# SafeRL-Lab/Massive-MARL-Benchmark

Measured on AMD Instinct MI355X. Metric: env-steps/sec (whole node), TenAnt 4096 envs/GPU, PPO rollout, higher is better.
Workload: dtype f32 (policy-layer products: fp32 operands as 2 row-scaled fp16 planes (kept to 2^-22), 3 f16 MFMA products, fp32 accumulation; error vs float64 <= the exact-fp32 MFMA kernel's, see policy_layers_error_vs_f64); 1 GPU; TenAnt num_envs=4096 per GPU, PPO rollout: ActorCritic MLP [1024,1024,512]x2 (fp32) + fused sim step (dt 0.0166, 2 substeps) + RolloutStorage + GAE every 8 steps; envs_per_gpu=4096, global_envs=4096, parallelism=env-sharded x1, no data-path collective, hipgraph=True, refresh_in_graph=True, rollouts_per_graph=1, fused_act_and_bound_slots=True, obs_planes_from_step_kernel=True, policy_head_in_step_kernel=True, critic_stream=True, critic_deferred=False, finite=True, resets_total=97569

## Files before the change

massive_marl_benchmark_amd/algorithms/rl/ppo/module.py:

```python
import ctypes
import math

import numpy as np
import torch
import torch.nn as nn

from .... import _lib


def get_activation(act_name):
    table = {"elu": nn.ELU, "selu": nn.SELU, "relu": nn.ReLU, "crelu": nn.ReLU, "lrelu": nn.LeakyReLU, "tanh": nn.Tanh,
             "sigmoid": nn.Sigmoid}
    if act_name not in table:
        print("invalid activation function!")
        return None
    return table[act_name]()


def _mlp(in_dim, hidden, out_dim, activation):
    layers, d = [], in_dim
    for h in hidden:
        layers += [nn.Linear(d, h), activation]
        d = h
    layers.append(nn.Linear(d, out_dim))
# ... 318 lines not shown
                continue
            x_planes[g0] = (bufs["x"][g0], bufs["xi"][g0], bufs["cs"][g0], bufs["ci"][g0])
            calls.append((L.mms_split_planes16_group, (idx, 1, M, x.shape[1], x.stride(0), arr([x]), arr([bufs["x"][g0]]), arr([bufs["xs"][g0]]), arr([bufs["xi"][g0]]),
                                                       nch, Lh if nch else 0, arr([chain]) if nch else None, arr([bufs["cs"][g0]]) if nch else None,
                                                       arr([bufs["ci"][g0]]) if nch else None, None, 0.0), "mms_split_planes16_group"))
            bufs["keep"].append(x)
        cur = [x_planes[src[g][0]][0] for g in range(G)]
        cur_inv = [x_planes[src[g][0]][1] for g in range(G)]
        for li in range(nl):
            last = li == nl - 1
            out = bufs["out"] if last else bufs["h"][li]
            ysc = None if last else arr([x_planes[src[g][0]][2][src[g][1], li] for g in range(G)])
            calls.append((L.mms_linear_group_act_split16, (idx, G, M, recs[0][li]["N"], recs[0][li]["K"], arr(cur), arr([recs[g][li]["planes"] for g in range(G)]),
                                                           arr([recs[g][li]["lin"].bias for g in range(G)]), arr(out), arr(cur_inv),
                                                           arr([recs[g][li]["inv"] for g in range(G)]), ysc, 1, 0 if last else 1, None, None, None, None, None, 0),
                          "mms_linear_group_act_split16"))
            if not last:
                cur, cur_inv = out, [x_planes[src[g][0]][3][src[g][1], li] for g in range(G)]
        return calls, bufs["out"]

    def _split_applies(self, M, lins, networks=2):
        if not (self.split_layers and M > 0 and M % 128 == 0 and all(l.out_features % 128 == 0 for l in lins)):
            return False
        need = self.split_min_tiles
        if need is None:
            dev = lins[0].weight.device
            need = torch.cuda.get_device_properties(dev).multi_processor_count if dev.type == "cuda" else 1
        return max(networks * (M // 128) * (l.out_features // 128) for l in lins) >= need

    def _split_hidden(self, nets, inputs, tag, planes=None):
        if self.split_format == "f16x2":
            return self._split_hidden16(nets, inputs, tag, planes)
        assert self.split_format == "bf16x3", self.split_format
        self._ensure_fresh()
        x0 = inputs[0]
        dev, M, K = x0.device, x0.shape[0], x0.shape[1]
        L, idx, stream = _lib.for_device(dev)
        G, nl = len(nets), len(nets[0])
        key = (tag, M, K, str(dev), G, tuple(l.out_features for l in nets[0]))
        if self._split_bufs is None:
            self._split_bufs = {}
        bufs = self._split_bufs.get(key)
        if bufs is None:
            u8 = lambda n: torch.empty(n, dtype=torch.uint8, device=dev)
            bufs = {"x": [u8(self._p32_bytes(M, K)) for _ in range(G)],
                    "h": [[u8(self._p32_bytes(M, l.out_features)) for _ in range(G)] for l in nets[0][:-1]],
                    "out": [torch.empty(M, nets[0][-1].out_features, device=dev) for _ in range(G)]}
            self._split_bufs[key] = bufs
        arr = lambda ts: (ctypes.c_void_p * len(ts))(*[t.data_ptr() for t in ts])
        cur = []
        for g, x in enumerate(inputs):
            same = next((h for h in range(g) if inputs[h].data_ptr() == x.data_ptr() and inputs[h].shape == x.shape), None)
            if same is not None:
                cur.append(cur[same])
                continue
            assert x.dtype == torch.float32 and x.stride(1) == 1
            _lib.check(L.mms_split_planes(idx, M, K, x.stride(0), ctypes.c_void_p(x.data_ptr()), ctypes.c_void_p(bufs["x"][g].data_ptr()), stream),
                       None, "mms_split_planes", L)
            cur.append(bufs["x"][g])
        for li in range(nl):
            lins = [net[li] for net in nets]
            last = li == nl - 1
            out = bufs["out"] if last else bufs["h"][li]
            wp = [self._weight_planes(l, L, idx, stream) for l in lins]
            _lib.check(L.mms_linear_group_act_split(idx, G, M, lins[0].out_features, lins[0].in_features, arr(cur), arr(wp),
                                                    arr([l.bias.detach() for l in lins]), arr(out), 1, 0 if last else 1, None, None, None, None, None, 0, stream),
                       None, "mms_linear_group_act_split", L)
            cur = out
        return bufs["out"]

    def _fused_hidden(self, x, critic_in, planes=None):
        a_lin = [m for m in self.actor if isinstance(m, nn.Linear)]
        c_lin = [m for m in self.critic if isinstance(m, nn.Linear)]
        if not self._fp32_layers_qualify():
            return None
        p = lambda t: ctypes.c_void_p(t.data_ptr())
        dev = x.device
        L, idx, stream = _lib.for_device(dev)
        ha, hc = x.contiguous(), critic_in.contiguous()
        M = ha.shape[0]
        if self._split_applies(M, a_lin[:-1]) and ha.data_ptr() % 16 == 0 and hc.data_ptr() % 16 == 0:
            out = self._split_hidden([a_lin[:-1], c_lin[:-1]], [ha, hc], "act", planes)
            return out[0], out[1]
        key = (M, str(dev))
        if self._act_bufs is None or self._act_bufs[0] != key:
            self._act_bufs = (key, [(torch.empty(M, la.out_features, device=dev), torch.empty(M, la.out_features, device=dev))
                                    for la in a_lin[:-1]])
        for (la, lc), (ya, yc) in zip(zip(a_lin[:-1], c_lin[:-1]), self._act_bufs[1]):
            _lib.check(L.mms_linear2_act(idx, M, la.out_features, la.in_features, p(ha), p(la.weight.detach()), p(la.bias.detach()), p(ya),
                                         p(hc), p(lc.weight.detach()), p(lc.bias.detach()), p(yc), 1, stream), None, "mms_linear2_act", L)
            ha, hc = ya, yc
        return ha, hc

    def _hidden_one(self, net, x):
        lin = [m for m in net if isinstance(m, nn.Linear)][:-1]
        L, idx, stream = _lib.for_device(x.device)
        p = lambda t: ctypes.c_void_p(t.data_ptr())
        M = x.shape[0]
        key = (M, str(x.device), id(net))
        if self._one_bufs is None or self._one_bufs[0] != key:
            self._one_bufs = (key, [torch.empty(M, l.out_features, device=x.device) for l in lin])
        h = x
        for l, y in zip(lin, self._one_bufs[1]):
            _lib.check(L.mms_linear2_act(idx, M, l.out_features, l.in_features, p(h), p(l.weight.detach()), p(l.bias.detach()), p(y),
                                         None, None, None, None, 1, stream), None, "mms_linear2_act", L)
            h = y
        return h

    def _actor_pass(self, x):
        last = self.actor[-1]
        if (self.fuse_head and x.is_cuda and isinstance(last, nn.Linear) and last.weight.dtype == torch.float32
                and last.in_features % 64 == 0 and last.out_features <= 128 and last.bias is not None):
            if self._trunk is None:
                self._trunk = [self.actor[:-1]]
            return None, self._trunk[0](x)
        return self.actor(x), None

    def _sample(self, mean, value, hidden=None, vhidden=None):
        src = mean if mean is not None else hidden
        N, A = src.shape[0], self.log_std.shape[0]
        dev = src.device
        L, idx, stream = _lib.for_device(dev)
        if self._counters is None or self._counters.numel() != N or self._counters.device != dev:
            self._counters = torch.zeros(N, dtype=torch.int64, device=dev)
        storage, actions_out = self._bound if self._bound is not None else (None, None)
        ckey = None
        if storage is not None and mean is None and value is None and hidden.is_contiguous() and (vhidden is None or vhidden.is_contiguous()):
            la, lc = self.actor[-1], self.critic[-1]
            ckey = (storage.actions.data_ptr(), storage.values.data_ptr(), storage.step, hidden.data_ptr(), None if vhidden is None else vhidden.data_ptr(),
                    None if actions_out is None else actions_out.data_ptr(), N, la.weight.data_ptr(), la.bias.data_ptr(), lc.weight.data_ptr(),
                    lc.bias.data_ptr(), self.log_std.data_ptr(), self._counters.data_ptr(), None if self._step_engine is None else id(self._step_engine))
            if self._sample_calls is None:
                self._sample_calls = {}
            hit = self._sample_calls.get(ckey)
            if hit is not None:
                args, ret, head = hit
                if head is not None and self._step_engine is not None:
                    self._step_engine.bind_policy_head(head)
                else:
                    _lib.check(L.mms_ppo_heads_act(*args, stream), None, "mms_ppo_heads_act", L)
                return ret
        if storage is not None:
            s = storage.step
            act, logp, val = storage.actions[s], storage.actions_log_prob[s], storage.values[s]
            mu, sigma = storage.mu[s], storage.sigma[s]
        else:
            act, mu, sigma = (torch.empty(N, A, device=dev) for _ in range(3))
            logp, val = torch.empty(N, 1, device=dev), torch.empty(N, 1, device=dev)
        p = lambda t: None if t is None else ctypes.c_void_p(t.data_ptr())
        value = None if value is None else value.contiguous().float()
        log_std = self.log_std.detach().float().contiguous()
        if mean is not None:
            mean = mean.contiguous().float()
            _lib.check(L.mms_ppo_act(idx, p(mean), p(value), p(log_std), self.seed, p(self._counters), self.row_offset, 1,
                                     p(actions_out), p(act), p(logp), p(val), p(mu), p(sigma), N, A, stream),
                       None, "mms_ppo_act", L)
        else:
            last = self.actor[-1]
            hidden = hidden.contiguous()
            vlast = self.critic[-1]
            vh = None if vhidden is None else vhidden.contiguous()
            args = (idx, p(hidden), p(last.weight.detach()), p(last.bias.detach()), last.in_features, p(value), p(vh),
                    None if vh is None else p(vlast.weight.detach()), None if vh is None else p(vlast.bias.detach()),
                    0 if vh is None else vlast.in_features, p(log_std), self.seed, p(self._counters), self.row_offset, 1,
                    p(actions_out), p(act), p(logp), p(val), p(mu), p(sigma), N, A)
            head = None
# ... 106 lines not shown
```

massive_marl_benchmark_amd/csrc/head_block.h:

```cpp
#pragma once
#include <hip/hip_runtime.h>
#ifndef MMS_HEAD_STAMP
#define MMS_HEAD_STAMP 0
#endif
#include <stdint.h>

#include "mms_lane.h"
#include "rollout_lane.h"

namespace mms {

struct PpoActOut {
    float* actions_out; float* act_slot; float* logp_slot; float* value_slot; float* mu_slot; float* sigma_slot;
    float* lds_actions = nullptr;
    int64_t lds_row0 = 0;
};
__device__ __forceinline__ void ppo_sample_row(const float* mean_row, const float* __restrict__ value, const float* __restrict__ log_std,
                                               uint64_t seed, int64_t* __restrict__ counters, int64_t row_offset, int ref_scale,
                                               const PpoActOut& o, int64_t row, int A, int lane, bool have_value = false, float value_now = 0.f) {
    const int64_t c = counters[row];
    float lp = 0.f;
    for (int j = lane; j < A; j += 64) {
        const float ls = log_std[j];
        const float m = mean_row[j];
        float term;
        const float act = ppo_sample_one(m, ls, seed, (uint64_t)(row_offset + row), (uint64_t)c, (uint32_t)j, ref_scale, term);
        lp += term;
        if (o.actions_out) o.actions_out[row * A + j] = act;
        if (o.lds_actions) o.lds_actions[(row - o.lds_row0) * A + j] = act;
        if (o.act_slot) o.act_slot[row * A + j] = act;
        if (o.mu_slot) o.mu_slot[row * A + j] = m;
        if (o.sigma_slot) o.sigma_slot[row * A + j] = ls;
    }
#pragma unroll
    for (int m = 32; m >= 1; m >>= 1) lp += __shfl_xor(lp, m, 64);
    if (lane == 0) {
        if (o.logp_slot) o.logp_slot[row] = lp;
        if (o.value_slot && (have_value || value)) o.value_slot[row] = have_value ? value_now : value[row];
        counters[row] = c + 1;
    }
}

typedef float f32x4 __attribute__((ext_vector_type(4)));

template <int NCT, int WAVES, int RT, int UB = 4, bool TILED = false>
__device__ __forceinline__ void ppo_head_block(float* s_part, const int tid, const bool active, const int64_t r0,
                                               const float* __restrict__ hidden, const float* __restrict__ weight,
                                               const float* __restrict__ bias, int H, const float* __restrict__ value,
                                               const float* __restrict__ vhidden, const float* __restrict__ vweight,
                                               const float* __restrict__ vbias, int VH,
                                               const float* __restrict__ log_std, uint64_t seed, int64_t* __restrict__ counters,
                                               int64_t row_offset, int ref_scale, const PpoActOut& o, int64_t N, int A,
                                               const float* __restrict__ weight_tiles = nullptr) {
    constexpr int AP = NCT * 16, ROWS = 16 * RT;
    constexpr int RPW = ROWS / WAVES;
#if MMS_HEAD_STAMP
    uint64_t st[6];
    st[0] = __builtin_amdgcn_s_memrealtime();
#define MMS_HEAD_ST(i) do { asm volatile("s_waitcnt vmcnt(0) lgkmcnt(0)" ::: "memory"); st[i] = __builtin_amdgcn_s_memrealtime(); } while (0)
#else
#define MMS_HEAD_ST(i) do { } while (0)
#endif
    const int lane = tid & 63, wave = active ? (tid >> 6) : 0;
    const int i = lane & 15, g = lane >> 4;
    float v_rows[RPW];
#pragma unroll
    for (int q = 0; q < RPW; q++) v_rows[q] = 0.f;
    if (active) {
        const float* hrow[RT];
#pragma unroll
        for (int rt = 0; rt < RT; rt++) {
            const int64_t row_a = r0 + 16 * rt + i < N ? r0 + 16 * rt + i : N - 1;
            hrow[rt] = hidden + row_a * (int64_t)H + 4 * g;
        }
        const float* wrow[NCT];
#pragma unroll
        for (int ct = 0; ct < NCT; ct++) {
            const int j = ct * 16 + i;
            wrow[ct] = weight + (int64_t)(j < A ? j : A - 1) * H + 4 * g;
        }
        f32x4 acc[RT][NCT];
#pragma unroll
        for (int rt = 0; rt < RT; rt++)
#pragma unroll
            for (int ct = 0; ct < NCT; ct++) acc[rt][ct] = f32x4{0.f, 0.f, 0.f, 0.f};
#pragma unroll
        for (int q = 0; q < RPW; q++) {
            const int64_t row = r0 + wave * RPW + q;
            if (vhidden && row < N) {
                const float* hv = vhidden + row * (int64_t)VH;
                float part = 0.f;
                for (int k = lane * 4; k < VH; k += 256) {
                    const float4 h4 = *reinterpret_cast<const float4*>(hv + k), w4 = *reinterpret_cast<const float4*>(vweight + k);
                    part += h4.x * w4.x + h4.y * w4.y + h4.z * w4.z + h4.w * w4.w;
                }
#pragma unroll
                for (int m = 32; m >= 1; m >>= 1) part += __shfl_xor(part, m, 64);
                v_rows[q] = part + vbias[0];
            }
        }
        MMS_HEAD_ST(1);
        const int kq = H / WAVES;
        const int kbeg = wave * kq;
        for (int kc = kbeg; kc < kbeg + kq; kc += 64) {
#pragma unroll
            for (int u0 = 0; u0 < 4; u0 += UB) {
                float4 a[RT][UB], b[UB][NCT];
#pragma unroll
                for (int u = 0; u < UB; u++) {
#pragma unroll
                    for (int rt = 0; rt < RT; rt++) a[rt][u] = *reinterpret_cast<const float4*>(hrow[rt] + kc + 16 * (u0 + u));
#pragma unroll
                    for (int ct = 0; ct < NCT; ct++)
                        b[u][ct] = TILED ? *reinterpret_cast<const float4*>(weight_tiles + ((size_t)(ct * (H / 4) + (kc / 4 + 4 * (u0 + u) + g)) * 16 + i) * 4)
                                         : *reinterpret_cast<const float4*>(wrow[ct] + kc + 16 * (u0 + u));
                }
#pragma unroll
                for (int rt = 0; rt < RT; rt++)
#pragma unroll
                    for (int u = 0; u < UB; u++) {
#pragma unroll
                        for (int ct = 0; ct < NCT; ct++) acc[rt][ct] = __builtin_amdgcn_mfma_f32_16x16x4f32(a[rt][u].x, b[u][ct].x, acc[rt][ct], 0, 0, 0);
#pragma unroll
                        for (int ct = 0; ct < NCT; ct++) acc[rt][ct] = __builtin_amdgcn_mfma_f32_16x16x4f32(a[rt][u].y, b[u][ct].y, acc[rt][ct], 0, 0, 0);
#pragma unroll
                        for (int ct = 0; ct < NCT; ct++) acc[rt][ct] = __builtin_amdgcn_mfma_f32_16x16x4f32(a[rt][u].z, b[u][ct].z, acc[rt][ct], 0, 0, 0);
#pragma unroll
                        for (int ct = 0; ct < NCT; ct++) acc[rt][ct] = __builtin_amdgcn_mfma_f32_16x16x4f32(a[rt][u].w, b[u][ct].w, acc[rt][ct], 0, 0, 0);
                    }
            }
        }
        MMS_HEAD_ST(2);
        float* mine = s_part + (size_t)wave * ROWS * AP;
#pragma unroll
        for (int rt = 0; rt < RT; rt++)
#pragma unroll
            for (int ct = 0; ct < NCT; ct++) {
#pragma unroll
                for (int r = 0; r < 4; r++) mine[(16 * rt + 4 * g + r) * AP + ct * 16 + i] = acc[rt][ct][r];
            }
    }
    __syncthreads();
    MMS_HEAD_ST(3);
    float* s_mean = s_part + (size_t)WAVES * ROWS * AP;
    if (active)
        for (int e = tid; e < ROWS * AP; e += 64 * WAVES) {
            const int j = e % AP;
            float sum = s_part[e];
#pragma unroll
            for (int w = 1; w < WAVES; w++) sum += s_part[w * ROWS * AP + e];
            s_mean[e] = sum + bias[j < A ? j : 0];
        }
    __syncthreads();
    MMS_HEAD_ST(4);
    if (active) {
#pragma unroll
        for (int q = 0; q < RPW; q++) {
            const int r = wave * RPW + q;
            const int64_t row = r0 + r;
            if (row >= N) continue;
            ppo_sample_row(s_mean + r * AP, value, log_std, seed, counters, row_offset, ref_scale, o, row, A, lane, vhidden != nullptr, v_rows[q]);
        }
    }
#if MMS_HEAD_STAMP
    MMS_HEAD_ST(5);
    if (r0 == 0 && tid == 0 && o.sigma_slot)
        for (int i = 1; i < 6; i++) o.sigma_slot[i] = 0.01f * (float)(st[i] - st[0]);
#endif
}

}
```

massive_marl_benchmark_amd/csrc/rollout_lane.h:

```cpp
#pragma once
#include "mms_lane.h"

namespace mms {

MMS_HD void gae_ppo_column(const float* rewards, const uint8_t* dones, const float* values, const float* last_values, float* returns,
                           float* advantages, int T, int64_t N, int64_t i, float gamma, float lam, double& sum, double& sq) {
    float adv = 0.f;
    float next_v = last_values[i];
    for (int t = T - 1; t >= 0; t--) {
        float v = values[t * N + i];
        float nt = 1.0f - (float)dones[t * N + i];
        float delta = rewards[t * N + i] + nt * gamma * next_v - v;
        adv = delta + nt * gamma * lam * adv;
        float ret = adv + v;
        returns[t * N + i] = ret;
        float a = ret - v;
        advantages[t * N + i] = a;
        sum += (double)a;
        sq += (double)a * (double)a;
        next_v = v;
    }
}
MMS_HD void adv_norm_params(const double* stats, float& mean, float& inv) {
    double n = stats[2];
    double m = stats[0] / n;
    double var = (stats[1] - n * m * m) / (n - 1.0);
    inv = (float)(1.0 / (sqrt(var > 0.0 ? var : 0.0) + 1e-8));
    mean = (float)m;
}
MMS_HD void gae_marl_column(const float* rewards, const float* value_preds, const float* masks, float* returns, int T, int64_t N, int64_t cols,
                            int64_t c, int64_t i, float gamma, float lam, int use_norm, float mean, float var) {
    float sd = 1.f;
    if (use_norm) sd = sqrtf(var); else mean = 0.f;
    float gae = 0.f;
    float v1 = value_preds[(int64_t)T * cols + c];
    if (use_norm) v1 = v1 * sd + mean;
    for (int t = T - 1; t >= 0; t--) {
        float v0 = value_preds[(int64_t)t * cols + c];
        if (use_norm) v0 = v0 * sd + mean;
        float m = masks[(int64_t)(t + 1) * N + i];
        float delta = rewards[(int64_t)t * N + i] + gamma * v1 * m - v0;
        gae = delta + gamma * lam * m * gae;
        returns[(int64_t)t * cols + c] = gae + v0;
        v1 = v0;
    }
}
MMS_HD int64_t marl_view_source(int64_t i, int agents, int per, int shared) {
    const int w = per + shared, row = agents * per + shared;
    int64_t e = i / ((int64_t)agents * w);
    int r = (int)(i - e * agents * w);
    int k = r / w, j = r - k * w;
    int src = (j < per) ? k * per + j : agents * per + (j - per);
    return e * row + src;
}
MMS_HD float ppo_sample_one(float mean, float log_std, uint64_t seed, uint64_t row_global, uint64_t counter, uint32_t j, int ref_scale, float& logp_term) {
    float scale, lscale;
    if (ref_scale) { float sd = expf(log_std); scale = sd * sd; lscale = logf(scale); }
    else { scale = expf(log_std); lscale = log_std; }
    const float z = rand_normal(seed, row_global, counter, j);
    logp_term = -0.5f * z * z - lscale - 0.9189385332046727f;
    return mean + scale * z;
}

}
```

massive_marl_benchmark_amd/csrc/step_kernels.hip:

```cpp
#include <hip/hip_runtime.h>

#include "head_block.h"
#include "mms_lane.h"
#include "step_args.h"

namespace mms {

template <int CTRL>
__device__ __forceinline__ float dpp_mov(float x) {
    return __builtin_bit_cast(float, __builtin_amdgcn_update_dpp(0, __builtin_bit_cast(int, x), CTRL, 0xF, 0xF, true));
}
__device__ __forceinline__ float quad_sum(float x) {
    x += dpp_mov<0xB1>(x);
    x += dpp_mov<0x4E>(x);
    return x;
}
__device__ __forceinline__ float oct_sum(float x) {
    x = quad_sum(x);
    x += dpp_mov<0x141>(x);
    return x;
}
__device__ __forceinline__ void quad_sum(Sym6& A, S6& p) {
#pragma unroll
    for (int k = 0; k < 21; k++) A.m[k] = quad_sum(A.m[k]);
// ... 4 lines not shown
#pragma unroll
    for (int k = 0; k < 9; k++) c.t[k] = oct_sum(c.t[k]);
}
__device__ __forceinline__ float wave_sum(float x) {
    x = oct_sum(x);
    x += dpp_mov<0x140>(x);
    x += __shfl_xor(x, 16, 64);
    x += __shfl_xor(x, 32, 64);
    return x;
}

typedef float f32x4_t __attribute__((ext_vector_type(4)));
__device__ __forceinline__ void stream_store(float4* dst, float4 v) {
    __builtin_nontemporal_store(f32x4_t{v.x, v.y, v.z, v.w}, reinterpret_cast<f32x4_t*>(dst));
}

__device__ __forceinline__ RigidState load_rigid(const float* r) {
    RigidState B;
    B.pos = V3{r[0], r[1], r[2]};
    B.qx = r[3]; B.qy = r[4]; B.qz = r[5]; B.qw = r[6];
    B.vel = V3{r[7], r[8], r[9]};
    B.ang = V3{r[10], r[11], r[12]};
    return B;
}
__device__ __forceinline__ void store_rigid(float* r, const RigidState& B) {
    r[0] = B.pos.x; r[1] = B.pos.y; r[2] = B.pos.z;
    r[3] = B.qx; r[4] = B.qy; r[5] = B.qz; r[6] = B.qw;
    r[7] = B.vel.x; r[8] = B.vel.y; r[9] = B.vel.z;
    r[10] = B.ang.x; r[11] = B.ang.y; r[12] = B.ang.z;
}

#ifndef MMS_WAVES_PER_EU
#define MMS_WAVES_PER_EU 2
#endif
__host__ __device__ inline size_t ant_env_lds_floats(int obs_dim, int A) {
    return (size_t)((obs_dim + 3) & ~3) + 16 + (sizeof(BoxPose) + 15) / 16 * 4 + 28 + 8 + (size_t)(((RP_STRIDE + 6) * A + 3) & ~3) +
           (size_t)((4 * A + 2 + 7 + 3) & ~3);
}
#ifndef MMS_WAVES_PER_EU_PACKED
#define MMS_WAVES_PER_EU_PACKED 3
#endif
template <int TASK, int BLOCK, int EPB, int AT, bool DR, bool HEAD = false>
#ifndef MMS_WAVES_PER_EU_WIDE
#define MMS_WAVES_PER_EU_WIDE 3
#endif
__global__ void __launch_bounds__(BLOCK, BLOCK == 64 ? MMS_WAVES_PER_EU : ((BLOCK == 192 || BLOCK == 768) ? MMS_WAVES_PER_EU_PACKED : MMS_WAVES_PER_EU_WIDE)) ant_step_kernel(StepArgs a) {
    extern __shared__ __attribute__((aligned(16))) float lds[];
    const mms_config* __restrict__ Cg = a.cfg;
    constexpr int kCfgFloats = (int)((sizeof(mms_config) + 15) / 16 * 4);
    static_assert(sizeof(mms_config) % 4 == 0, "copied word by word");
    const mms_config* C = reinterpret_cast<const mms_config*>(lds);
    const mms_model* M = &C->model;
    float2 ac_head = make_float2(0.f, 0.f);
    constexpr int kObsAT = TASK == MMS_TASK_TEN_ANT ? 38 * AT + 8 : (TASK == MMS_TASK_MULTI_ANT_CIRCLE ? 38 * AT : 60);
    constexpr int kPrevAT = TASK == MMS_TASK_TEN_ANT ? 4 * AT + 2 : (TASK == MMS_TASK_MULTI_ANT_CIRCLE ? 2 * AT : 6);
    const int obs_dim = AT > 0 ? kObsAT : a.obs_dim;
    const int prev_dim = AT > 0 ? kPrevAT : a.prev_dim;
    const int obs_pad = (obs_dim + 3) & ~3;

    const int A = AT > 0 ? AT : a.num_agents;
    const int LA = 4 * A;
    const int ant_region = EPB * LA;
    const int box_region = (BLOCK == 512 && EPB == 1 && ant_region <= 448) ? 448 : ((ant_region + 7) & ~7);
    const int bt = (int)threadIdx.x - box_region;
    const bool is_ant = (int)threadIdx.x < ant_region;
    const bool is_box = bt >= 0 && bt < 8 * EPB;
    const int e_loc = EPB == 1 ? 0 : (is_ant ? (int)threadIdx.x / LA : (is_box ? bt >> 3 : 0));
    const int tid = is_ant ? (int)threadIdx.x - e_loc * LA : 0;
    const int corner = bt & 7;
    const bool box_lead = is_box && corner == 0;
    const int env_raw = blockIdx.x * EPB + e_loc;
    const bool live = env_raw < a.num_envs;
    const int env = live ? env_raw : a.num_envs - 1;
    const int ant = tid >> 2, leg = tid & 3;

    LegConst* s_leg = reinterpret_cast<LegConst*>(lds + kCfgFloats);
    constexpr int kBoxOff = 0, kBpOff = 16, kFacOff = kBpOff + (int)((sizeof(BoxPose) + 15) / 16 * 4), kEpiOff = kFacOff + 28, kRedOff = kEpiOff + 8;
    const size_t env_stride = (ant_env_lds_floats(obs_dim, A) + 3) & ~(size_t)3;
    float* lds_envs = lds + kCfgFloats + (4 * sizeof(LegConst) + 15) / 16 * 4;
    float* s_root = lds_envs + (size_t)EPB * ((ant_env_lds_floats(AT > 0 ? kObsAT : a.obs_dim, A) + 3) & ~(size_t)3);
    constexpr bool kStage = AT > 0 && ((EPB * (AT + 1) * 13) % 4) == 0;
    const int root_floats = kStage ? EPB * (A + 1) * 13 : 0;
    float* lds_lanes = s_root + ((root_floats + 3) & ~3);
    if constexpr (HEAD) {
        static_assert(BLOCK == 768 && EPB == 16 && AT == 10 && TASK == MMS_TASK_TEN_ANT && kStage, "the fused head assumes 16 rows x 80 actions per block");
        float* s_head = lds_lanes;
        float* s_head_actions = s_head + 9 * 16 * 80;
        static_assert((9 + 1) * 16 * 80 <= 6 * 4 * BLOCK, "the head's LDS must fit the parking space");
        if (threadIdx.x >= 512) {
            const int t = (int)threadIdx.x - 512;
            const float4* src = reinterpret_cast<const float4*>(a.root_states + (size_t)blockIdx.x * root_floats);
            for (int i = t; i < root_floats / 4; i += 256) reinterpret_cast<float4*>(s_root)[i] = src[i];
            for (int i = t; i < (int)(sizeof(mms_config) / 4); i += 256) lds[i] = reinterpret_cast<const float*>(Cg)[i];
            if (t < 4) s_leg[t] = load_leg_const(&Cg->model, t);
            constexpr int kStageOff = ((kRedOff + (RP_STRIDE + 6) * AT + 3) & ~3) + ((kObsAT + 3) & ~3);
            for (int i = t; i < EPB * prev_dim; i += 256) {
                const int e = i / prev_dim, k = i - e * prev_dim;
                (lds_envs + (size_t)e * env_stride + kStageOff)[k] = a.prev[((size_t)blockIdx.x * EPB + e) * prev_dim + k];
            }
        }
        PpoActOut o{a.head.actions_out, a.head.act_slot, a.head.logp_slot, a.head.value_slot, a.head.mu_slot, a.head.sigma_slot};
        o.lds_actions = s_head_actions;
        o.lds_row0 = (int64_t)blockIdx.x * 16;
        if (a.head.weight_tiles)
            ppo_head_block<5, 8, 1, 4, true>(s_head, (int)threadIdx.x, threadIdx.x < 512, (int64_t)blockIdx.x * 16, a.head.hidden, a.head.weight, a.head.bias, a.head.H, nullptr,
                                             a.head.vhidden, a.head.vweight, a.head.vbias, a.head.VH, a.head.log_std, a.head.seed, a.head.counters, a.head.row_offset,
                                             a.head.reference_scale, o, a.num_envs, 8 * AT, a.head.weight_tiles);
        else
            ppo_head_block<5, 8, 1, 4>(s_head, (int)threadIdx.x, threadIdx.x < 512, (int64_t)blockIdx.x * 16, a.head.hidden, a.head.weight, a.head.bias, a.head.H, nullptr,
                                       a.head.vhidden, a.head.vweight, a.head.vbias, a.head.VH, a.head.log_std, a.head.seed, a.head.counters, a.head.row_offset,
                                       a.head.reference_scale, o, a.num_envs, 8 * AT);
        __syncthreads();
        if (threadIdx.x < 16 * 4 * AT) ac_head = reinterpret_cast<const float2*>(s_head_actions)[threadIdx.x];
    }
    const KinPark park{lds_lanes + 4 * threadIdx.x, 4 * BLOCK};
    LegDR* s_dr = reinterpret_cast<LegDR*>(lds_lanes + 6 * 4 * BLOCK) + threadIdx.x;
    float* env_lds = lds_envs + (size_t)e_loc * env_stride;
    float* s_box = env_lds + kBoxOff;
    BoxPose* s_bp = reinterpret_cast<BoxPose*>(env_lds + kBpOff);
    float4* s_fac = reinterpret_cast<float4*>(env_lds + kFacOff);
    float* s_epi = env_lds + kEpiOff;
    float* s_red = env_lds + kRedOff;
    float* s_wr = s_red + RP_STRIDE * A;
    float* s_obs = env_lds + ((kRedOff + (RP_STRIDE + 6) * A + 3) & ~3);
    float* s_stage = s_obs + obs_pad;
    float* s_act = s_obs + (TASK != MMS_TASK_ONE_ANT ? 38 * ant + 30 + 2 * leg : 52 + 2 * leg);

    const int actors = A + 1;
    const bool reset_now = a.reset[env] != 0;

    AntLane S = {};
    float2 ac = make_float2(0.f, 0.f);
    if (kStage && !HEAD) {
        const size_t g0 = (size_t)blockIdx.x * root_floats, gtot = (size_t)a.num_envs * actors * 13;
        if (g0 + root_floats <= gtot) {
            const float4* src = reinterpret_cast<const float4*>(a.root_states + g0);
            for (int i = threadIdx.x; i < root_floats / 4; i += BLOCK) reinterpret_cast<float4*>(s_root)[i] = src[i];
        } else {
            for (int i = threadIdx.x; i < root_floats; i += BLOCK) {
                size_t f = g0 + i;
                if (f >= gtot) f = gtot - (size_t)actors * 13 + (f % ((size_t)actors * 13));
                s_root[i] = a.root_states[f];
            }
        }
    } else if (is_ant) {
        const float* r = a.root_states + ((size_t)env * actors + ant) * 13;
        S.pos = V3{r[0], r[1], r[2]};
        S.qx = r[3]; S.qy = r[4]; S.qz = r[5]; S.qw = r[6];
        S.vel = V3{r[7], r[8], r[9]};
        S.ang = V3{r[10], r[11], r[12]};
    }
    if (is_ant) {
        float4 d = reinterpret_cast<const float4*>(a.dof_state + (size_t)env * A * 16)[tid];
        S.q[0] = d.x; S.qd[0] = d.y; S.q[1] = d.z; S.qd[1] = d.w;
        if constexpr (HEAD) ac = ac_head;
        else ac = reinterpret_cast<const float2*>(a.actions + (size_t)env * A * 8)[tid];
        if (DR) *s_dr = load_leg_dr(a.dr + ((size_t)env * A + ant) * MMS_DR_FLOATS, leg);
    }
    for (int i = threadIdx.x; i < (HEAD ? 0 : (int)(sizeof(mms_config) / 4)); i += BLOCK) lds[i] = reinterpret_cast<const float*>(Cg)[i];
    if (!HEAD && threadIdx.x < 4) s_leg[threadIdx.x] = load_leg_const(&Cg->model, threadIdx.x);

    for (int i = threadIdx.x; i < (HEAD ? 0 : EPB * prev_dim); i += BLOCK) {
        const int e = i / prev_dim, k = i - e * prev_dim;
        const int en = min((int)(blockIdx.x * EPB + e), a.num_envs - 1);
        (lds_envs + (size_t)e * env_stride + (s_stage - env_lds))[k] = a.prev[(size_t)en * prev_dim + k];
    }
    if (is_box && corner == 1) {
        s_stage[prev_dim + 0] = a.env_origin[3 * env]; s_stage[prev_dim + 1] = a.env_origin[3 * env + 1];
        s_stage[prev_dim + 2] = a.env_origin[3 * env + 2];
        int64_t pr = a.progress[env], rc = a.reset_count[env];
        int* si = reinterpret_cast<int*>(s_stage + prev_dim + 3);
        si[0] = (int)(pr & 0xffffffff); si[1] = (int)(pr >> 32); si[2] = (int)(rc & 0xffffffff); si[3] = (int)(rc >> 32);
    }
    if (is_ant) {
        s_act[0] = clampf(ac.x, -Cg->clip_actions, Cg->clip_actions);
        s_act[1] = clampf(ac.y, -Cg->clip_actions, Cg->clip_actions);
    }
    if (kStage) __syncthreads();
    if (kStage && is_ant) {
        const float* r = s_root + (e_loc * actors + ant) * 13;
        S.pos = V3{r[0], r[1], r[2]};
        S.qx = r[3]; S.qy = r[4]; S.qz = r[5]; S.qw = r[6];
        S.vel = V3{r[7], r[8], r[9]};
        S.ang = V3{r[10], r[11], r[12]};
    }
    if (box_lead) {
        RigidState B0 = load_rigid(kStage ? s_root + (e_loc * actors + A) * 13 : a.root_states + ((size_t)env * actors + A) * 13);
        store_rigid(s_box, B0);
        s_bp->pos = B0.pos; s_bp->R = quat_to_mat(B0.qx, B0.qy, B0.qz, B0.qw); s_bp->v = B0.vel; s_bp->w = B0.ang;
        const mms_model* Mb = kStage ? &C->model : &Cg->model;
        s_bp->half = V3{Mb->box_half[0], Mb->box_half[1], Mb->box_half[2]};
    }
    __syncthreads();
    const LegConst& L = s_leg[leg];
    float sens[6] = {0.f, 0.f, 0.f, 0.f, 0.f, 0.f};
    if (TASK == MMS_TASK_ONE_ANT && is_ant) {
        const float* fs = a.foot_sensors + ((size_t)env * A + ant) * 24 + 6 * leg;
#pragma unroll
        for (int i = 0; i < 6; i++) sens[i] = fs[i];
    }

    const bool simulate = a.do_physics && !reset_now;
    if (a.do_physics) {
        const float h = C->dt / (float)C->substeps;
        constexpr bool kSensors = (TASK == MMS_TASK_ONE_ANT);
        constexpr bool kOneWave = (BLOCK == 64 && EPB == 1);
        auto ant_phase = [&](bool wait_for_box) -> S6 {
            S6 wr = S6{V3{0, 0, 0}, V3{0, 0, 0}};
            Sym6 IA0;
            S6 pA0;
            LegPass P;
            SensorPass SP;
            LegInward W;
            constexpr bool kSplit = BLOCK > 64;
            if (kSplit && is_ant && simulate) leg_inward_open<kSensors, DR>(M, L, h, S, P, &SP, W, park, s_dr);
            if (kSplit ? wait_for_box : false) __syncthreads();
            if (is_ant && simulate) {
                const float tau1 = s_act[0] * L.gear[0] * C->power_scale;
                const float tau2 = s_act[1] * L.gear[1] * C->power_scale;
                if (!kSplit) leg_inward<kSensors, DR>(M, L, h, S, leg, tau1, tau2, true, *s_bp, P, &SP, IA0, pA0, park, s_dr);
                else leg_inward_close<kSensors, DR>(M, L, h, S, leg, tau1, tau2, true, *s_bp, P, &SP, IA0, pA0, W, s_dr);
            }
            quad_sum(IA0, pA0);
            if (is_ant && simulate) leg_outward<kSensors>(M, L, h, S, leg, *s_bp, P, &SP, IA0, pA0, wr, sens, park);
            return wr;
        };
        auto stage_wrench = [&](S6 wr) {
            wr.a.x = quad_sum(wr.a.x); wr.a.y = quad_sum(wr.a.y); wr.a.z = quad_sum(wr.a.z);
            wr.l.x = quad_sum(wr.l.x); wr.l.y = quad_sum(wr.l.y); wr.l.z = quad_sum(wr.l.z);
            if (is_ant && leg == 0) {
                s_wr[0 * A + ant] = wr.a.x; s_wr[1 * A + ant] = wr.a.y; s_wr[2 * A + ant] = wr.a.z;
                s_wr[3 * A + ant] = wr.l.x; s_wr[4 * A + ant] = wr.l.y; s_wr[5 * A + ant] = wr.l.z;
            }
        };
        auto gather_wrench = [&]() -> S6 {
            float t = 0.f;
            if (corner < 6) {
                const float* col = s_wr + corner * A;
                for (int i = 0; i < A; i++) t += col[i];
            }
#define MMS_FROM(c) __int_as_float(__builtin_amdgcn_ds_swizzle(__float_as_int(t), 0x18 | ((c) << 5)))
            return S6{V3{MMS_FROM(0), MMS_FROM(1), MMS_FROM(2)}, V3{MMS_FROM(3), MMS_FROM(4), MMS_FROM(5)}};
#undef MMS_FROM
        };
        auto box_store = [&](const RigidState& B) {
            store_rigid(s_box, B);
            s_bp->pos = B.pos; s_bp->R = quat_to_mat(B.qx, B.qy, B.qz, B.qw); s_bp->v = B.vel; s_bp->w = B.ang;
        };
        const bool box_friction = M->boxgnd_mu > 0.f;
        for (int s = 0; s < C->substeps; s++) {
            S6 wr = ant_phase(s > 0);
            BoxCorner bc = {};
            if (is_box && !box_friction) {
                bc = box_corner(M, h, load_rigid(s_box), s_bp->R, corner);
                oct_sum(bc);
            }
            if (is_box && box_friction) {
                const RigidState B0 = load_rigid(s_box);
                BoxCornerF bf = box_corner_friction(M, h, B0, s_bp->R, corner);
// ... 401 lines not shown
```

Before: 26.92 million env-steps/s.

## Overlap head noise draws and critic dot products with the action-head MFMA

In the fused step kernel with the policy head, waves 0-7 run the action-head matrix product. Waves 8-11 now do more than stage roots and config: they also compute the critic values (four rows per wave, with a 512-wide specialised path), draw the Gaussian noise and log-probs, and stage bias, env origin, reset flag and dof state into registers or LDS. Mean assembly and sampling then finish after a single reduction, so the critic and RNG work no longer serialises with the MFMA. The cost is more register pressure and extra barriers, and the module gains a freshness check on the non-split hidden path.

```diff
diff --git a/massive_marl_benchmark_amd/algorithms/rl/ppo/module.py b/massive_marl_benchmark_amd/algorithms/rl/ppo/module.py
--- a/massive_marl_benchmark_amd/algorithms/rl/ppo/module.py
+++ b/massive_marl_benchmark_amd/algorithms/rl/ppo/module.py
@@ -424,6 +424,7 @@
         if self._split_applies(M, a_lin[:-1]) and ha.data_ptr() % 16 == 0 and hc.data_ptr() % 16 == 0:
             out = self._split_hidden([a_lin[:-1], c_lin[:-1]], [ha, hc], "act", planes)
             return out[0], out[1]
+        self._ensure_fresh()
         key = (M, str(dev))
         if self._act_bufs is None or self._act_bufs[0] != key:
             self._act_bufs = (key, [(torch.empty(M, la.out_features, device=dev), torch.empty(M, la.out_features, device=dev))
diff --git a/massive_marl_benchmark_amd/csrc/head_block.h b/massive_marl_benchmark_amd/csrc/head_block.h
--- a/massive_marl_benchmark_amd/csrc/head_block.h
+++ b/massive_marl_benchmark_amd/csrc/head_block.h
@@ -43,6 +43,150 @@
 
 typedef float f32x4 __attribute__((ext_vector_type(4)));
 
+struct PpoRowDraw { int64_t c; float z[2], scale[2], ls[2], lp; };
+__device__ __forceinline__ PpoRowDraw ppo_draw_row(const float* __restrict__ log_std, uint64_t seed, const int64_t* __restrict__ counters,
+                                                   int64_t row_offset, int ref_scale, int64_t row, int A, int lane) {
+    PpoRowDraw d;
+    d.c = counters[row];
+    float lp = 0.f;
+#pragma unroll
+    for (int s = 0; s < 2; s++) {
+        const int j = lane + 64 * s;
+        d.z[s] = d.scale[s] = d.ls[s] = 0.f;
+        if (j < A) {
+            float term;
+            d.ls[s] = log_std[j];
+            d.z[s] = ppo_sample_noise(d.ls[s], seed, (uint64_t)(row_offset + row), (uint64_t)d.c, (uint32_t)j, ref_scale, d.scale[s], term);
+            lp += term;
+        }
+    }
+#pragma unroll
+    for (int m = 32; m >= 1; m >>= 1) lp += __shfl_xor(lp, m, 64);
+    d.lp = lp;
+    return d;
+}
+__device__ __forceinline__ void ppo_finish_row(const float* mean_row, const PpoRowDraw& d, int64_t* __restrict__ counters, const PpoActOut& o,
+                                               int64_t row, int A, int lane) {
+#pragma unroll
+    for (int s = 0; s < 2; s++) {
+        const int j = lane + 64 * s;
+        if (j < A) {
+            const float m = mean_row[j];
+            const float act = m + d.scale[s] * d.z[s];
+            if (o.actions_out) o.actions_out[row * A + j] = act;
+            if (o.lds_actions) o.lds_actions[(row - o.lds_row0) * A + j] = act;
+            if (o.act_slot) o.act_slot[row * A + j] = act;
+            if (o.mu_slot) o.mu_slot[row * A + j] = m;
+            if (o.sigma_slot) o.sigma_slot[row * A + j] = d.ls[s];
+        }
+    }
+    if (lane == 0) {
+        if (o.logp_slot) o.logp_slot[row] = d.lp;
+        counters[row] = d.c + 1;
+    }
+}
+
+__device__ __forceinline__ float ppo_critic_row(const float* __restrict__ vhidden, const float* __restrict__ vweight, const float* __restrict__ vbias,
+                                                int VH, int64_t row, int lane) {
+    const float* hv = vhidden + row * (int64_t)VH;
+    float part = 0.f;
+    for (int k = lane * 4; k < VH; k += 256) {
+        const float4 h4 = *reinterpret_cast<const float4*>(hv + k), w4 = *reinterpret_cast<const float4*>(vweight + k);
+        part += h4.x * w4.x + h4.y * w4.y + h4.z * w4.z + h4.w * w4.w;
+    }
+#pragma unroll
+    for (int m = 32; m >= 1; m >>= 1) part += __shfl_xor(part, m, 64);
+    return part + vbias[0];
+}
+template <int R>
+__device__ __forceinline__ void ppo_critic_rows(float (&v)[R], const float* __restrict__ vhidden, const float* __restrict__ vweight,
+                                                const float* __restrict__ vbias, int VH, int64_t row0, int lane) {
+    if (VH == 512) {
+        float4 w4[2], h4[R][2];
+#pragma unroll
+        for (int n = 0; n < 2; n++) w4[n] = *reinterpret_cast<const float4*>(vweight + lane * 4 + 256 * n);
+#pragma unroll
+        for (int q = 0; q < R; q++)
+#pragma unroll
+            for (int n = 0; n < 2; n++) h4[q][n] = *reinterpret_cast<const float4*>(vhidden + (row0 + q) * 512 + lane * 4 + 256 * n);
+#pragma unroll
+        for (int q = 0; q < R; q++) {
+            float part = 0.f;
+#pragma unroll
+            for (int n = 0; n < 2; n++) part += h4[q][n].x * w4[n].x + h4[q][n].y * w4[n].y + h4[q][n].z * w4[n].z + h4[q][n].w * w4[n].w;
+#pragma unroll
+            for (int m = 32; m >= 1; m >>= 1) part += __shfl_xor(part, m, 64);
+            v[q] = part + vbias[0];
+        }
+    } else {
+#pragma unroll
+        for (int q = 0; q < R; q++) v[q] = ppo_critic_row(vhidden, vweight, vbias, VH, row0 + q, lane);
+    }
+}
+
+
+template <int NCT, int WAVES, int RT, int UB, bool TILED>
+__device__ __forceinline__ void ppo_head_matrix(float* s_part, const int wave, const int lane, const int64_t r0, const float* __restrict__ hidden,
+                                                const float* __restrict__ weight, int H, int64_t N, int A, const float* __restrict__ weight_tiles) {
+    constexpr int AP = NCT * 16, ROWS = 16 * RT;
+    const int i = lane & 15, g = lane >> 4;
+    const float* hrow[RT];
+#pragma unroll
+    for (int rt = 0; rt < RT; rt++) {
+        const int64_t row_a = r0 + 16 * rt + i < N ? r0 + 16 * rt + i : N - 1;
+        hrow[rt] = hidden + row_a * (int64_t)H + 4 * g;
+    }
+    const float* wrow[NCT];
+#pragma unroll
+    for (int ct = 0; ct < NCT; ct++) {
+        const int j = ct * 16 + i;
+        wrow[ct] = weight + (int64_t)(j < A ? j : A - 1) * H + 4 * g;
+    }
+    f32x4 acc[RT][NCT];
+#pragma unroll
+    for (int rt = 0; rt < RT; rt++)
+#pragma unroll
+        for (int ct = 0; ct < NCT; ct++) acc[rt][ct] = f32x4{0.f, 0.f, 0.f, 0.f};
+    const int kq = H / WAVES;
+    const int kbeg = wave * kq;
+    for (int kc = kbeg; kc < kbeg + kq; kc += 64) {
+#pragma unroll
+        for (int u0 = 0; u0 < 4; u0 += UB) {
+            float4 a[RT][UB], b[UB][NCT];
+#pragma unroll
+            for (int u = 0; u < UB; u++) {
+#pragma unroll
+                for (int rt = 0; rt < RT; rt++) a[rt][u] = *reinterpret_cast<const float4*>(hrow[rt] + kc + 16 * (u0 + u));
+#pragma unroll
+                for (int ct = 0; ct < NCT; ct++)
+                    b[u][ct] = TILED ? *reinterpret_cast<const float4*>(weight_tiles + ((size_t)(ct * (H / 4) + (kc / 4 + 4 * (u0 + u) + g)) * 16 + i) * 4)
+                                     : *reinterpret_cast<const float4*>(wrow[ct] + kc + 16 * (u0 + u));
+            }
+#pragma unroll
+            for (int rt = 0; rt < RT; rt++)
+#pragma unroll
+                for (int u = 0; u < UB; u++) {
+#pragma unroll
+                    for (int ct = 0; ct < NCT; ct++) acc[rt][ct] = __builtin_amdgcn_mfma_f32_16x16x4f32(a[rt][u].x, b[u][ct].x, acc[rt][ct], 0, 0, 0);
+#pragma unroll
+                    for (int ct = 0; ct < NCT; ct++) acc[rt][ct] = __builtin_amdgcn_mfma_f32_16x16x4f32(a[rt][u].y, b[u][ct].y, acc[rt][ct], 0, 0, 0);
+#pragma unroll
+                    for (int ct = 0; ct < NCT; ct++) acc[rt][ct] = __builtin_amdgcn_mfma_f32_16x16x4f32(a[rt][u].z, b[u][ct].z, acc[rt][ct], 0, 0, 0);
+#pragma unroll
+                    for (int ct = 0; ct < NCT; ct++) acc[rt][ct] = __builtin_amdgcn_mfma_f32_16x16x4f32(a[rt][u].w, b[u][ct].w, acc[rt][ct], 0, 0, 0);
+                }
+        }
+    }
+    float* mine = s_part + (size_t)wave * ROWS * AP;
+#pragma unroll
+    for (int rt = 0; rt < RT; rt++)
+#pragma unroll
+        for (int ct = 0; ct < NCT; ct++) {
+#pragma unroll
+            for (int r = 0; r < 4; r++) mine[(16 * rt + 4 * g + r) * AP + ct * 16 + i] = acc[rt][ct][r];
+        }
+}
+
 template <int NCT, int WAVES, int RT, int UB = 4, bool TILED = false>
 __device__ __forceinline__ void ppo_head_block(float* s_part, const int tid, const bool active, const int64_t r0,
                                                const float* __restrict__ hidden, const float* __restrict__ weight,
@@ -62,83 +206,18 @@
 #define MMS_HEAD_ST(i) do { } while (0)
 #endif
     const int lane = tid & 63, wave = active ? (tid >> 6) : 0;
-    const int i = lane & 15, g = lane >> 4;
     float v_rows[RPW];
 #pragma unroll
     for (int q = 0; q < RPW; q++) v_rows[q] = 0.f;
     if (active) {
-        const float* hrow[RT];
-#pragma unroll
-        for (int rt = 0; rt < RT; rt++) {
-            const int64_t row_a = r0 + 16 * rt + i < N ? r0 + 16 * rt + i : N - 1;
-            hrow[rt] = hidden + row_a * (int64_t)H + 4 * g;
-        }
-        const float* wrow[NCT];
-#pragma unroll
-        for (int ct = 0; ct < NCT; ct++) {
-            const int j = ct * 16 + i;
-            wrow[ct] = weight + (int64_t)(j < A ? j : A - 1) * H + 4 * g;
-        }
-        f32x4 acc[RT][NCT];
-#pragma unroll
-        for (int rt = 0; rt < RT; rt++)
-#pragma unroll
-            for (int ct = 0; ct < NCT; ct++) acc[rt][ct] = f32x4{0.f, 0.f, 0.f, 0.f};
 #pragma unroll
         for (int q = 0; q < RPW; q++) {
             const int64_t row = r0 + wave * RPW + q;
-            if (vhidden && row < N) {
-                const float* hv = vhidden + row * (int64_t)VH;
-                float part = 0.f;
-                for (int k = lane * 4; k < VH; k += 256) {
-                    const float4 h4 = *reinterpret_cast<const float4*>(hv + k), w4 = *reinterpret_cast<const float4*>(vweight + k);
-                    part += h4.x * w4.x + h4.y * w4.y + h4.z * w4.z + h4.w * w4.w;
-                }
-#pragma unroll
-                for (int m = 32; m >= 1; m >>= 1) part += __shfl_xor(part, m, 64);
-                v_rows[q] = part + vbias[0];
-            }
+            if (vhidden && row < N) v_rows[q] = ppo_critic_row(vhidden, vweight, vbias, VH, row, lane);
         }
         MMS_HEAD_ST(1);
-        const int kq = H / WAVES;
-        const int kbeg = wave * kq;
-        for (int kc = kbeg; kc < kbeg + kq; kc += 64) {
-#pragma unroll
-            for (int u0 = 0; u0 < 4; u0 += UB) {
-                float4 a[RT][UB], b[UB][NCT];
-#pragma unroll
-                for (int u = 0; u < UB; u++) {
-#pragma unroll
-                    for (int rt = 0; rt < RT; rt++) a[rt][u] = *reinterpret_cast<const float4*>(hrow[rt] + kc + 16 * (u0 + u));
-#pragma unroll
-                    for (int ct = 0; ct < NCT; ct++)
-                        b[u][ct] = TILED ? *reinterpret_cast<const float4*>(weight_tiles + ((size_t)(ct * (H / 4) + (kc / 4 + 4 * (u0 + u) + g)) * 16 + i) * 4)
-                                         : *reinterpret_cast<const float4*>(wrow[ct] + kc + 16 * (u0 + u));
-                }
-#pragma unroll
-                for (int rt = 0; rt < RT; rt++)
-#pragma unroll
-                    for (int u = 0; u < UB; u++) {
-#pragma unroll
-                        for (int ct = 0; ct < NCT; ct++) acc[rt][ct] = __builtin_amdgcn_mfma_f32_16x16x4f32(a[rt][u].x, b[u][ct].x, acc[rt][ct], 0, 0, 0);
-#pragma unroll
-                        for (int ct = 0; ct < NCT; ct++) acc[rt][ct] = __builtin_amdgcn_mfma_f32_16x16x4f32(a[rt][u].y, b[u][ct].y, acc[rt][ct], 0, 0, 0);
-#pragma unroll
-                        for (int ct = 0; ct < NCT; ct++) acc[rt][ct] = __builtin_amdgcn_mfma_f32_16x16x4f32(a[rt][u].z, b[u][ct].z, acc[rt][ct], 0, 0, 0);
-#pragma unroll
-                        for (int ct = 0; ct < NCT; ct++) acc[rt][ct] = __builtin_amdgcn_mfma_f32_16x16x4f32(a[rt][u].w, b[u][ct].w, acc[rt][ct], 0, 0, 0);
-                    }
-            }
-        }
+        ppo_head_matrix<NCT, WAVES, RT, UB, TILED>(s_part, wave, lane, r0, hidden, weight, H, N, A, weight_tiles);
         MMS_HEAD_ST(2);
-        float* mine = s_part + (size_t)wave * ROWS * AP;
-#pragma unroll
-        for (int rt = 0; rt < RT; rt++)
-#pragma unroll
-            for (int ct = 0; ct < NCT; ct++) {
-#pragma unroll
-                for (int r = 0; r < 4; r++) mine[(16 * rt + 4 * g + r) * AP + ct * 16 + i] = acc[rt][ct][r];
-            }
     }
     __syncthreads();
     MMS_HEAD_ST(3);
diff --git a/massive_marl_benchmark_amd/csrc/rollout_lane.h b/massive_marl_benchmark_amd/csrc/rollout_lane.h
--- a/massive_marl_benchmark_amd/csrc/rollout_lane.h
+++ b/massive_marl_benchmark_amd/csrc/rollout_lane.h
@@ -53,12 +53,17 @@
     int src = (j < per) ? k * per + j : agents * per + (j - per);
     return e * row + src;
 }
-MMS_HD float ppo_sample_one(float mean, float log_std, uint64_t seed, uint64_t row_global, uint64_t counter, uint32_t j, int ref_scale, float& logp_term) {
-    float scale, lscale;
+MMS_HD float ppo_sample_noise(float log_std, uint64_t seed, uint64_t row_global, uint64_t counter, uint32_t j, int ref_scale, float& scale, float& logp_term) {
+    float lscale;
     if (ref_scale) { float sd = expf(log_std); scale = sd * sd; lscale = logf(scale); }
     else { scale = expf(log_std); lscale = log_std; }
     const float z = rand_normal(seed, row_global, counter, j);
     logp_term = -0.5f * z * z - lscale - 0.9189385332046727f;
+    return z;
+}
+MMS_HD float ppo_sample_one(float mean, float log_std, uint64_t seed, uint64_t row_global, uint64_t counter, uint32_t j, int ref_scale, float& logp_term) {
+    float scale;
+    const float z = ppo_sample_noise(log_std, seed, row_global, counter, j, ref_scale, scale, logp_term);
     return mean + scale * z;
 }
 
diff --git a/massive_marl_benchmark_amd/csrc/step_kernels.hip b/massive_marl_benchmark_amd/csrc/step_kernels.hip
--- a/massive_marl_benchmark_amd/csrc/step_kernels.hip
+++ b/massive_marl_benchmark_amd/csrc/step_kernels.hip
@@ -110,34 +110,70 @@
     constexpr bool kStage = AT > 0 && ((EPB * (AT + 1) * 13) % 4) == 0;
     const int root_floats = kStage ? EPB * (A + 1) * 13 : 0;
     float* lds_lanes = s_root + ((root_floats + 3) & ~3);
+    float4 dof_head = make_float4(0.f, 0.f, 0.f, 0.f);
+    int64_t reset_head = 0;
     if constexpr (HEAD) {
         static_assert(BLOCK == 768 && EPB == 16 && AT == 10 && TASK == MMS_TASK_TEN_ANT && kStage, "the fused head assumes 16 rows x 80 actions per block");
         float* s_head = lds_lanes;
+        float* s_head_mean = s_head + 8 * 16 * 80;
         float* s_head_actions = s_head + 9 * 16 * 80;
-        static_assert((9 + 1) * 16 * 80 <= 6 * 4 * BLOCK, "the head's LDS must fit the parking space");
-        if (threadIdx.x >= 512) {
+        float* s_head_bias = s_head + 10 * 16 * 80;
+        static_assert(10 * 16 * 80 + 80 <= 6 * 4 * BLOCK, "the head's LDS must fit the parking space");
+        const int64_t r0 = (int64_t)blockIdx.x * 16;
+        reset_head = a.reset[env];
+        if (is_ant) dof_head = reinterpret_cast<const float4*>(a.dof_state + (size_t)env * A * 16)[tid];
+        PpoActOut o{a.head.actions_out, a.head.act_slot, a.head.logp_slot, a.head.value_slot, a.head.mu_slot, a.head.sigma_slot};
+        o.lds_actions = s_head_actions;
+        o.lds_row0 = r0;
+        const int lane = (int)threadIdx.x & 63, w8 = ((int)threadIdx.x - 512) >> 6;
+        PpoRowDraw draw[4];
+        if (threadIdx.x < 512) {
+            if (a.head.weight_tiles)
+                ppo_head_matrix<5, 8, 1, 4, true>(s_head, (int)threadIdx.x >> 6, lane, r0, a.head.hidden, a.head.weight, a.head.H, a.num_envs, 8 * AT, a.head.weight_tiles);
+            else
+                ppo_head_matrix<5, 8, 1, 4, false>(s_head, (int)threadIdx.x >> 6, lane, r0, a.head.hidden, a.head.weight, a.head.H, a.num_envs, 8 * AT, nullptr);
+        } else {
             const int t = (int)threadIdx.x - 512;
             const float4* src = reinterpret_cast<const float4*>(a.root_states + (size_t)blockIdx.x * root_floats);
             for (int i = t; i < root_floats / 4; i += 256) reinterpret_cast<float4*>(s_root)[i] = src[i];
             for (int i = t; i < (int)(sizeof(mms_config) / 4); i += 256) lds[i] = reinterpret_cast<const float*>(Cg)[i];
             if (t < 4) s_leg[t] = load_leg_const(&Cg->model, t);
+            if (t < 8 * AT) s_head_bias[t] = a.head.bias[t];
             constexpr int kStageOff = ((kRedOff + (RP_STRIDE + 6) * AT + 3) & ~3) + ((kObsAT + 3) & ~3);
             for (int i = t; i < EPB * prev_dim; i += 256) {
                 const int e = i / prev_dim, k = i - e * prev_dim;
                 (lds_envs + (size_t)e * env_stride + kStageOff)[k] = a.prev[((size_t)blockIdx.x * EPB + e) * prev_dim + k];
             }
-        }
-        PpoActOut o{a.head.actions_out, a.head.act_slot, a.head.logp_slot, a.head.value_slot, a.head.mu_slot, a.head.sigma_slot};
-        o.lds_actions = s_head_actions;
-        o.lds_row0 = (int64_t)blockIdx.x * 16;
-        if (a.head.weight_tiles)
-            ppo_head_block<5, 8, 1, 4, true>(s_head, (int)threadIdx.x, threadIdx.x < 512, (int64_t)blockIdx.x * 16, a.head.hidden, a.head.weight, a.head.bias, a.head.H, nullptr,
-                                             a.head.vhidden, a.head.vweight, a.head.vbias, a.head.VH, a.head.log_std, a.head.seed, a.head.counters, a.head.row_offset,
-                                             a.head.reference_scale, o, a.num_envs, 8 * AT, a.head.weight_tiles);
-        else
-            ppo_head_block<5, 8, 1, 4>(s_head, (int)threadIdx.x, threadIdx.x < 512, (int64_t)blockIdx.x * 16, a.head.hidden, a.head.weight, a.head.bias, a.head.H, nullptr,
-                                       a.head.vhidden, a.head.vweight, a.head.vbias, a.head.VH, a.head.log_std, a.head.seed, a.head.counters, a.head.row_offset,
-                                       a.head.reference_scale, o, a.num_envs, 8 * AT);
+            if (is_box && corner == 1) {
+                float* st = lds_envs + (size_t)e_loc * env_stride + kStageOff;
+                st[prev_dim + 0] = a.env_origin[3 * env]; st[prev_dim + 1] = a.env_origin[3 * env + 1];
+                st[prev_dim + 2] = a.env_origin[3 * env + 2];
+                int64_t pr = a.progress[env], rc = a.reset_count[env];
+                int* si = reinterpret_cast<int*>(st + prev_dim + 3);
+                si[0] = (int)(pr & 0xffffffff); si[1] = (int)(pr >> 32); si[2] = (int)(rc & 0xffffffff); si[3] = (int)(rc >> 32);
+            }
+            if (a.head.vhidden) {
+                float v[4];
+                ppo_critic_rows<4>(v, a.head.vhidden, a.head.vweight, a.head.vbias, a.head.VH, r0 + 4 * w8, lane);
+                if (lane == 0 && o.value_slot)
+#pragma unroll
+                    for (int q = 0; q < 4; q++) o.value_slot[r0 + 4 * w8 + q] = v[q];
+            }
+#pragma unroll
+            for (int q = 0; q < 4; q++)
+                draw[q] = ppo_draw_row(a.head.log_std, a.head.seed, a.head.counters, a.head.row_offset, a.head.reference_scale, r0 + 4 * w8 + q, 8 * AT, lane);
+        }
+        __syncthreads();
+        for (int e = threadIdx.x; e < 16 * 80; e += BLOCK) {
+            float sum = s_head[e];
+#pragma unroll
+            for (int w = 1; w < 8; w++) sum += s_head[w * 16 * 80 + e];
+            s_head_mean[e] = sum + s_head_bias[e % 80];
+        }
+        __syncthreads();
+        if (threadIdx.x >= 512)
+#pragma unroll
+            for (int q = 0; q < 4; q++) ppo_finish_row(s_head_mean + (4 * w8 + q) * 80, draw[q], a.head.counters, o, r0 + 4 * w8 + q, 8 * AT, lane);
         __syncthreads();
         if (threadIdx.x < 16 * 4 * AT) ac_head = reinterpret_cast<const float2*>(s_head_actions)[threadIdx.x];
     }
@@ -155,7 +191,7 @@
     float* s_act = s_obs + (TASK != MMS_TASK_ONE_ANT ? 38 * ant + 30 + 2 * leg : 52 + 2 * leg);
 
     const int actors = A + 1;
-    const bool reset_now = a.reset[env] != 0;
+    const bool reset_now = (HEAD ? reset_head : a.reset[env]) != 0;
 
     AntLane S = {};
     float2 ac = make_float2(0.f, 0.f);
@@ -179,7 +215,7 @@
         S.ang = V3{r[10], r[11], r[12]};
     }
     if (is_ant) {
-        float4 d = reinterpret_cast<const float4*>(a.dof_state + (size_t)env * A * 16)[tid];
+        float4 d = HEAD ? dof_head : reinterpret_cast<const float4*>(a.dof_state + (size_t)env * A * 16)[tid];
         S.q[0] = d.x; S.qd[0] = d.y; S.q[1] = d.z; S.qd[1] = d.w;
         if constexpr (HEAD) ac = ac_head;
         else ac = reinterpret_cast<const float2*>(a.actions + (size_t)env * A * 8)[tid];
@@ -193,7 +229,7 @@
         const int en = min((int)(blockIdx.x * EPB + e), a.num_envs - 1);
         (lds_envs + (size_t)e * env_stride + (s_stage - env_lds))[k] = a.prev[(size_t)en * prev_dim + k];
     }
-    if (is_box && corner == 1) {
+    if (!HEAD && is_box && corner == 1) {
         s_stage[prev_dim + 0] = a.env_origin[3 * env]; s_stage[prev_dim + 1] = a.env_origin[3 * env + 1];
         s_stage[prev_dim + 2] = a.env_origin[3 * env + 2];
         int64_t pr = a.progress[env], rc = a.reset_count[env];
@@ -201,8 +237,9 @@
         si[0] = (int)(pr & 0xffffffff); si[1] = (int)(pr >> 32); si[2] = (int)(rc & 0xffffffff); si[3] = (int)(rc >> 32);
     }
     if (is_ant) {
-        s_act[0] = clampf(ac.x, -Cg->clip_actions, Cg->clip_actions);
-        s_act[1] = clampf(ac.y, -Cg->clip_actions, Cg->clip_actions);
+        const mms_config* Cc = HEAD ? C : Cg;
+        s_act[0] = clampf(ac.x, -Cc->clip_actions, Cc->clip_actions);
+        s_act[1] = clampf(ac.y, -Cc->clip_actions, Cc->clip_actions);
     }
     if (kStage) __syncthreads();
     if (kStage && is_ant) {
```

Result: faster. 27.19 million env-steps/s (median of 6 runs) (+1.0%).
